# DJjjjhao/FIRA-ICSE

Hardware: AMD Instinct MI355X
Metric: training commits/sec (FIRA default config) (higher is better)
Workload: dtype f32; 1 GPU; BASELINE configs[1]: FIRA training step (fwd+bwd+Adam, dropout 0.1/0.2), batch 32 commits/GPU, fp32, 650-node graphs (mean nnz 1066/graph), vocab 24650; global_batch=32, parallelism=dp1

## Files before the change

### fira_icse_amd/csrc/engine.h

```cpp
#pragma once
#include "common.h"
#include <string>
#include <vector>

namespace fira {

int gemm_f32(hipStream_t s, int tA, int tB, int M, int N, int K, const float* A, int lda, const float* B, int ldb,
             float* C, int ldc, const float* bias, int flags, int splitk);
int gemm_f32_ex(hipStream_t s, int tA, int tB, int M, int N, int K, const float* A, int lda, const float* B, int ldb,
                float* C, int ldc, const float* bias, int flags, int splitk, float* colsum,
                const int32_t* c_rows = nullptr, const float* relu_mask = nullptr);
int gemm_bf16_ex(hipStream_t s, int tA, int tB, int M, int N, int K, const float* A, int lda, const float* B, int ldb,
                 float* C, int ldc, const float* bias, int flags, int splitk, float* colsum,
                 const int32_t* c_rows = nullptr, const float* relu_mask = nullptr);
struct ShadowEntry { int64_t offset; int rows, cols, pitch_t; int64_t offset_t; };
constexpr int SHADOW_MAX = 64;
struct ShadowTable {
    int n = 0;
    int64_t wbt_elems = 0;
    int tile_start[SHADOW_MAX + 1] = {0};
    ShadowEntry e[SHADOW_MAX];
};
int weight_shadows(hipStream_t s, const ShadowTable& tab, const float* P, uint16_t* Wb, uint16_t* WbT);
int gemm_bf16_wb_ex(hipStream_t s, int M, int N, int K, const float* A, int lda, const uint16_t* Bb, int ldb, float* C,
                    int ldc, const float* bias, int flags, int splitk, const int32_t* c_rows = nullptr,
                    const float* relu_mask = nullptr);
int gemm_bf16_group_add_wgrad(hipStream_t s, int M, int N, int K, const float* A, int lda, const float* B, int ldb,
                              float* C, int ldc, float* colsum, int max_split = 0);
int gemm_bf16_group_flush(hipStream_t s);
bool gemm_bf16_takes(int M, int N, int K);
void gemm_bf16_group_reset();
bool gemm_bf16_group_full();
bool gemm_wgrad_panel_takes(int M, int N, int K, const float* A, int lda, const float* B, int ldb, int ldc);
void gemm_wgrad_panel_reset();
bool gemm_wgrad_panel_full();
int gemm_wgrad_panel_pending();
int gemm_wgrad_panel_add(int M, int N, int K, const float* A, int lda, const float* B, int ldb, float* C, int ldc, float* colsum);
int gemm_wgrad_panel_flush(hipStream_t s, int np);
void gemm_wgrad_panel_scratch(float* buf, size_t n_floats);
int gemm_wgrad_panel(hipStream_t s, int np, int M, int N, int K, const float* A, int lda, const float* B, int ldb, float* C,
                     int ldc, float* colsum);
int gemm_group_add_wgrad(hipStream_t s, int M, int N, int K, const float* A, int lda, const float* B, int ldb, float* C,
                         int ldc, float* colsum, int max_split = 0);
int gemm_group_flush(hipStream_t s);
void gemm_group_reset();
bool gemm_group_full();
void gemm_set_pad_stream(hipStream_t s);
struct EpiRes;
bool gemm_tile32_takes(int tB, int M, int N, int K, const float* A, int lda, const float* B, int ldb);
bool gemm_tile32_try(hipStream_t s, int tB, int M, int N, int K, const float* A, int lda, const float* B, int ldb,
                     float* C, int ldc, const float* bias, int flags, int* rc, const int32_t* c_rows,
                     const float* relu_mask, const int32_t* a_rows, const EpiRes* er);
bool gemm_tile32_ln_try(hipStream_t s, int M, int N, const float* S, int lds, const float* W, const float* bias, float* Y,
                        int ldy, int flags, const float* gamma, const float* beta, float* x_out, float* stats_out, int* rc);
int gemm_tile32_lnb_blocks(int M);
bool gemm_tile32_lnb_try(hipStream_t s, int M, int N, const float* dy, const float* W, int ldw, float* dX, int lddx,
                         const float* relu_mask, const float* sum, const float* stats, const float* gamma, float* ds,
                         float* dx_drop, float* part, float dropout, uint64_t seed, uint32_t site, int* rc,
                         uint32_t idx0 = 0);
bool gemm_small_try(hipStream_t s, int tA, int tB, int M, int N, int K, const float* A, int lda, const float* B, int ldb,
                    float* C, int ldc, const float* bias, int flags, int* rc, const int32_t* c_rows = nullptr,
                    const float* relu_mask = nullptr);
int csr_spmm(hipStream_t s, int n_rows, const int32_t* rowptr, const int32_t* col, const float* val, const float* X,
             int ldx, float* Y, int ldy, int graph_rows, int variant);
int csr_spmm_ex(hipStream_t s, int n_rows, const int32_t* rowptr, const int32_t* col, const float* val, const float* X,
                int ldx, float* Y, int ldy, int graph_rows, int variant, int accum, float* rowsum);
int gcn_fused_fwd(hipStream_t s, int n_rows, const int32_t* rowptr, const int32_t* col, const float* val, const float* X,
                  const float* Wk, const float* bias, const float* r1_col, const float* gamma, const float* beta, float* sum,
                  float* y, float* stats, float* rowsum_out, const int32_t* slot2, float* y2, float dropout, uint64_t seed,
                  uint32_t site, int bf16, const uint16_t* Wx = nullptr);
int gcn_fused_bwd(hipStream_t s, int n_rows, const int32_t* rowptr, const int32_t* col, const float* val, const float* dY,
                  const float* Wk, float* u_out, float* acc_out, int bf16, const uint16_t* Wx = nullptr);
int gcn_split_planes(hipStream_t s, int n, const float* const* src, uint16_t* const* dst);
size_t head_logits_x3_scratch_elems(int R);
int head_logits_x3(hipStream_t s, int R, int V, const float* x, int ldx, const float* W, const float* bias, float* out, int ldo,
                   uint16_t* xplanes);
int transpose256(hipStream_t s, int nl, const float* W, float* Wt);
int linear_x3(hipStream_t s, int M, const float* X, int ldx, const uint16_t* Wx, int nb, const float* bias, float* out, int ldo,
              bool one_plane);
int split_planes_t(hipStream_t s, const float* W, int V, uint16_t* planes, bool one_plane);
int dgrad_x3_splitk(hipStream_t s, int M, int K, const float* A, int lda, const uint16_t* Wx, float* out, int ldo, bool one_plane);
int linear_x3_kacc(hipStream_t s, int M, const float* A, int lda, const uint16_t* Wx, int nkb, float* out, int ldo, bool accum,
                   bool one_plane);
int comb_fused_fwd(hipStream_t s, int n_rows, const float* Xc, const float* WqT, const float* WkT, const float* WoT,
                   const float* bqk, const float* bo, const float* vtab, int ldv, const int32_t* mark, float* qk, float* c,
                   const float* gamma, const float* beta, float* sum, float* y, const int32_t* y_rows, float* stats,
                   float dropout, uint64_t seed, uint32_t site_gate, uint32_t site_out, int bf16, const uint16_t* Wx = nullptr);
int comb_fused_bwd_parts();
int comb_fused_bwd(hipStream_t s, int n_rows, float* dG, const int32_t* rows, const float* sum, const float* stats,
                   const float* gamma, const float* Wo, const float* Wqk, const float* qk, const float* vtab, int ldv,
                   const int32_t* mark, float* dYc, float* dqk, float* part_ln, float* part_v, float dropout, uint64_t seed,
                   uint32_t site_gate, uint32_t site_out, int bf16, const uint16_t* WTx = nullptr);
struct TransposeTable { int n = 0; const float* src[24]; float* dst[24]; };
int transpose256_table(hipStream_t s, const TransposeTable& tab);
int embed_gather_fwd(hipStream_t s, int B, int L, const int32_t* idx, const float* table, const float* pos, float* out,
                     int out_bstride, int out_off);
int embed_grouped_bwd(hipStream_t s, int n_items, const int32_t* item_tok, const int32_t* item_ptr, const int32_t* rows,
                      float* dtable, const float* dnode);
int embed_list_bwd_small(hipStream_t s, int n, const int32_t* rows, const int32_t* ids, float* dtable, const float* dnode,
                         int table_rows);
int embed_gather_bwd(hipStream_t s, int B, int L, const int32_t* idx, float* dtable, const float* dout,
                     int out_bstride, int out_off, int padding_idx);
int embed_gather_bwd_small(hipStream_t s, int B, int L, const int32_t* idx, float* dtable, const float* dout,
                           int out_bstride, int out_off, int padding_idx, int table_rows);
int combination_fwd(hipStream_t s, int M, const float* qk, const float* vtab, int ldv, const int32_t* mark, float* out,
                    float dropout, uint64_t seed, uint32_t site);
int combination_bwd(hipStream_t s, int M, const float* qk, const float* vtab, int ldv, const int32_t* mark,
                    const float* dout, float* dqk, float* dvtab, int lddv, float dropout, uint64_t seed, uint32_t site,
                    float* part = nullptr);
int combination_bwd_blocks(int M);
struct RedEntry { float* dst; const float* src; int width, n_part, stride; };
constexpr int RED_MAX = 96;
struct RedTable {
    int n = 0;
    int wg_start[RED_MAX + 1] = {0};
    RedEntry e[RED_MAX];
};
int deferred_reduce(hipStream_t s, RedTable& tab);
int add_layernorm_fwd(hipStream_t s, int M, float* x, const float* res, const float* gamma, const float* beta,
                      float* y, float* stats, float dropout, uint64_t seed, uint32_t site, const int32_t* y_rows, const float* r1_row = nullptr,
                      const float* r1_col = nullptr,
                      const int32_t* slot2 = nullptr, float* y2 = nullptr,
// ... 170 lines not shown
```

### fira_icse_amd/csrc/engine.hip

```cpp
#include "engine.h"
#include <hip/hip_ext.h>
#include "epilogue.h"
#include <stdlib.h>
#include <map>
#include <mutex>

namespace fira {

static int64_t shadow_wbt_elems(const Layout& L);

struct Arena {
    char* base;
    size_t used = 0;
    explicit Arena(void* b) : base((char*)b) {}
    template <typename T>
    T* get(size_t n) {
        size_t bytes = (n * sizeof(T) + 255) / 256 * 256;
        T* p = base ? (T*)(base + used) : nullptr;
        used += bytes;
        return p;
    }
    float* f(size_t n) { return get<float>(n); }
};

// ... 45 lines not shown
    float* red_buf = nullptr;
    size_t red_cap = 0;
    float* panel_scratch = nullptr;
    size_t panel_floats = 0;
    float *dmem_c, *dsrc, *dsrc_c, *dtgt, *dkv_all, *ddec, *ddec_c, *dT_a, *dT_c;

    size_t build(void* ws, const fira_dims& d, int B_, bool training) {
        Arena a(ws);
        B = B_; L = d.sou_len; S = d.sub_len; A = d.ast_len; T = d.tar_len; V = d.vocab; nl = d.n_layer; F = d.d_ff;
        N = L + S + A;
        NB = B * N; CB = B * L; MB = B * (L + S); TB = B * T;
        ldl = (V + 63) / 64 * 64;
        const size_t D = FIRA_D;
        pos_code = a.f((size_t)L * D);
        pos_tar = a.f((size_t)T * D);
        mem_valid = a.get<int32_t>((size_t)MB);
        tar_valid = a.get<int32_t>((size_t)TB);
        compact_row = a.get<int32_t>((size_t)TB);
        iota = a.get<int32_t>((size_t)TB);
        row_bt = a.get<int32_t>((size_t)TB);
        rows_c = a.get<int32_t>((size_t)TB);
        code_slot = a.get<int32_t>((size_t)NB);
        mem_slot = a.get<int32_t>((size_t)NB);
        mem_off = a.get<int32_t>((size_t)B + 1);
        mem_valid_c = a.get<int32_t>((size_t)MB);
        inv_ntok = a.f(64);
        {
            const Layout* lay = get_layout(&d);
            const size_t tot = lay ? (size_t)lay->total : 0;
            wb = a.get<uint16_t>(tot);
            wbt = a.get<uint16_t>((lay ? (size_t)shadow_wbt_elems(*lay) : 0) + 64);
            w21b = a.get<uint16_t>((size_t)nl * D * D);
            w21bt = a.get<uint16_t>((size_t)nl * D * D + 64);
        }
        X.resize(nl + 1);
        for (int l = 0; l <= nl; ++l) X[l] = a.f((size_t)NB * D);
        enc.resize(nl);
        for (int l = 0; l < nl; ++l) {
            EncSave& e = enc[l];
            e.Xc = a.f((size_t)CB * D); e.qk = a.f((size_t)CB * 2 * D); e.c = a.f((size_t)CB * D);
            e.s1 = a.f((size_t)CB * D); e.st1 = a.f((size_t)CB * 2);
            e.Z = a.f((size_t)NB * D); e.s2 = a.f((size_t)NB * D); e.st2 = a.f((size_t)NB * 2);
        }
        vtab_all = a.f((size_t)4 * nl * D);
        W21 = a.f((size_t)nl * D * D); c21 = a.f((size_t)nl * D); rsum = a.f((size_t)NB);
        W21t = a.f((size_t)nl * D * D);
        W21x = a.get<uint16_t>((size_t)nl * 3 * D * D);
        W21tx = a.get<uint16_t>((size_t)nl * 3 * D * D);
        WcX = a.get<uint16_t>((size_t)nl * 9 * D * D);
        WcTX = a.get<uint16_t>((size_t)nl * 9 * D * D);
        WkvX = a.get<uint16_t>((size_t)nl * 6 * D * D);
        WkvT = a.f((size_t)nl * 2 * D * D);
        WkvTX = a.get<uint16_t>((size_t)nl * 6 * D * D);
        WoutTX = a.get<uint16_t>((size_t)cdiv(V, D) * 3 * D * D);
        xh_planes = a.get<uint16_t>(head_logits_x3_scratch_elems(TB));
        WcT = a.f((size_t)nl * 3 * D * D);
        H = a.f((size_t)NB * D);
        mem = a.f((size_t)MB * D);
        mem_c = a.f((size_t)MB * D);
        src_c = a.f((size_t)MB * D);
        x0 = a.f((size_t)TB * D);
        kvp = nl * 2 * D + KV_ROW_PAD;
        kv_all = a.f((size_t)MB * kvp);
        dec.resize(nl);
        for (int l = 0; l < nl; ++l) {
            DecSave& e = dec[l];
            e.qkv = a.f((size_t)TB * 3 * D); e.ao = a.f((size_t)TB * D); e.s_a = a.f((size_t)TB * D);
            e.st_a = a.f((size_t)TB * 2); e.x_a = a.f((size_t)TB * D); e.qc = a.f((size_t)TB * D);
            e.ao2 = a.f((size_t)TB * D); e.s_c = a.f((size_t)TB * D); e.st_c = a.f((size_t)TB * 2);
            e.x_c = a.f((size_t)TB * D); e.h = a.f((size_t)TB * F); e.s_f = a.f((size_t)TB * D);
            e.st_f = a.f((size_t)TB * 2); e.x_f = a.f((size_t)TB * D);
        }
        src = a.f((size_t)MB * D); tgt = a.f((size_t)TB * D);
        score = a.f((size_t)TB * (L + S)); gate = a.f((size_t)TB * 2);
        dec_c = a.f((size_t)TB * D); logits = a.f((size_t)TB * ldl);
        if (training) {
            dXa = a.f((size_t)NB * D); dXb = a.f((size_t)NB * D); dNB2 = a.f((size_t)NB * D);
            dCB_a = a.f((size_t)CB * D);
            red_cap = (size_t)nl * ((size_t)cdiv(NB, 16) * 4 * D + (size_t)cdiv(CB, 16) * 2 * D)
                    + (size_t)3 * nl * cdiv(TB, 16) * 2 * D
                    + (size_t)nl * std::max((size_t)cdiv(CB, 16) * 4 * D, (size_t)comb_fused_bwd_parts() * 6 * D + 64)
                    + (size_t)cdiv(L + S, 16) * B * COPY_PART_STRIDE + 4096;
            red_buf = a.f(red_cap);
            panel_floats = (size_t)320 * 256 * 256;
            panel_scratch = a.f(panel_floats);
            zero_beg = (float*)a.get<char>(0);
            dvtab_all = a.f((size_t)4 * nl * D);
            dW21 = a.f((size_t)nl * D * D + (size_t)nl * D); dc21 = dW21 + (size_t)nl * D * D;
            dtgt = a.f((size_t)TB * D);
            ddec_c = a.f((size_t)TB * D);
            zero_end = (float*)a.get<char>(0);
            dmem_c = a.f((size_t)MB * D); dsrc = a.f((size_t)MB * D); dsrc_c = a.f((size_t)MB * D);
            dkv_all = a.f((size_t)MB * kvp);
            ddec = a.f((size_t)TB * D);
            dT_a = a.f((size_t)TB * D); dT_c = a.f((size_t)TB * D);
            encg.resize(nl);
            decg.resize(nl);
            for (int l = 0; l < nl; ++l) {
                EncGrad& g = encg[l];
                g.dY2 = a.f((size_t)NB * D); g.dYc = a.f((size_t)CB * D);
                g.dqk = a.f((size_t)CB * 2 * D);
                DecGrad& h = decg[l];
                h.dYf = a.f((size_t)TB * D); h.dh = a.f((size_t)TB * F); h.dYc = a.f((size_t)TB * D);
                h.dq = a.f((size_t)TB * D); h.dYs = a.f((size_t)TB * D); h.dqkv = a.f((size_t)TB * 3 * D);
            }
        }
        return a.used;
    }
};

#define TRY(x)                 \
    do {                       \
        if (int e__ = (x)) return e__; \
    } while (0)

static int zero(hipStream_t s, void* p, size_t bytes) {
    hipError_t e = hipMemsetAsync(p, 0, bytes, s);
    if (e != hipSuccess) return set_err("hipMemsetAsync: %s", hipGetErrorString(e));
    return 0;
}

static thread_local int g_dtype = 0;
static thread_local int g_lanes = 1;
struct DtypeScope {
    int prev;
    explicit DtypeScope(int d) : prev(g_dtype) { g_dtype = d; }
    ~DtypeScope() { g_dtype = prev; }
};
static thread_local const float* g_P = nullptr;
static thread_local int64_t g_total = 0;
static thread_local const uint16_t* g_Wb = nullptr;
static thread_local const uint16_t* g_WbT = nullptr;
static thread_local const ShadowTable* g_tab = nullptr;
static thread_local const float* g_W21 = nullptr;
static thread_local int64_t g_W21n = 0;
static thread_local const uint16_t* g_W21b = nullptr;
static thread_local const uint16_t* g_W21bT = nullptr;

static const ShadowTable* shadow_table(const Layout& L) {
    static std::mutex mu;
    static std::map<const Layout*, ShadowTable*> cache;
    std::lock_guard<std::mutex> g(mu);
    auto it = cache.find(&L);
    if (it != cache.end()) return it->second;
    ShadowTable* t = new ShadowTable();
    const int D = FIRA_D;
    auto add = [&](int64_t off, int rows, int cols) {
        if (t->n == SHADOW_MAX) return;
        const int pitch = (rows + 7) / 8 * 8;
        t->e[t->n] = ShadowEntry{off, rows, cols, pitch, t->wbt_elems};
        t->wbt_elems += ((int64_t)cols * pitch + 63) / 64 * 64;
        t->tile_start[t->n + 1] = t->tile_start[t->n] + cdiv(rows, 64) * cdiv(cols, 64);
        ++t->n;
    };
    for (int l = 0; l < L.d.n_layer; ++l) {
        add(L.enc[l].wqk, 2 * D, D);
        add(L.enc[l].wo, D, D);
        add(L.dec[l].wqkv, 3 * D, D);
        add(L.dec[l].wo_s, D, D);
        add(L.dec[l].wq_c, D, D);
        add(L.dec[l].wo_c, D, D);
        add(L.dec[l].w1, L.d.d_ff, D);
        add(L.dec[l].w2, D, L.d.d_ff);
    }
    add(L.wkv_all, L.d.n_layer * 2 * D, D);
    add(L.wout, L.d.vocab, D);
    add(L.ws, D, D);
    add(L.wt, D, D);
// ... 1776 lines not shown
```

### fira_icse_amd/csrc/gemm_wgrad_panel.hip

```cpp
#include "engine.h"
#include "epilogue.h"
#include <algorithm>
#include <stdlib.h>

namespace fira {

typedef __bf16 pbf16x8 __attribute__((ext_vector_type(8)));
typedef __bf16 pbf16x2 __attribute__((ext_vector_type(2)));
typedef float pf32x2 __attribute__((ext_vector_type(2)));
typedef float pf32x16 __attribute__((ext_vector_type(16)));

constexpr int PN_T = 256;
constexpr int PN_KB = 16;
constexpr int PN_PART = PN_T * 32;
constexpr int PANEL_MAX = 48;

struct PanelProblem {
    const float *A, *B;
    float *C, *colsum;
    float* part;
    int M, N, K, lda, ldb, ldc;
    int tiles_m, tiles_n, slabs, k_slab;
};
struct PanelTable {
    int n;
    int wg_start[PANEL_MAX + 1];
    PanelProblem p[PANEL_MAX];
};

__device__ __forceinline__ int pn_unit(int row, int kh) { return kh * PN_T + row; }

__device__ __forceinline__ uint32_t pn_pack(float a, float b) {
    pf32x2 v = {a, b};
    return __builtin_bit_cast(uint32_t, __builtin_convertvector(v, pbf16x2));
}
__device__ __forceinline__ void pn_rest(float& a, float& b, uint32_t pk) {
    a -= __builtin_bit_cast(float, pk << 16);
    b -= __builtin_bit_cast(float, pk & 0xffff0000u);
}

__device__ __forceinline__ void pn_barrier() { asm volatile("s_waitcnt lgkmcnt(0)\n\ts_barrier" ::: "memory"); }

template <int NP>
__global__ __launch_bounds__(512) void wgrad_panel_kernel(const PanelTable tab) {
    extern __shared__ __attribute__((aligned(16))) char pn_lds[];
    __shared__ float pn_cs[PN_T];
    const int t = threadIdx.x, lane = t & 63, wave = __builtin_amdgcn_readfirstlane(t >> 6);
    int pi = 0;
    while (pi + 1 < tab.n && (int)blockIdx.x >= tab.wg_start[pi + 1]) ++pi;
    const PanelProblem& q = tab.p[pi];
    int w = blockIdx.x - tab.wg_start[pi];
    const int z = w % q.slabs;
    w /= q.slabs;
    const int tn = w % q.tiles_n, tm = w / q.tiles_n;
    const int m0 = tm * PN_T, n0 = tn * PN_T;
    const int k_beg = z * q.k_slab, k_end = min(q.K, k_beg + q.k_slab);
    const int nstep = (k_end - k_beg + PN_KB - 1) / PN_KB;
    const int opnd = t >> 8, idx = t & 255, kb = idx >> 7, cb = idx & 127;
    const float* src = opnd ? q.B : q.A;
    const int ld = opnd ? q.ldb : q.lda;
    const int c0 = (opnd ? n0 : m0) + 2 * cb;
    const int c_lim = opnd ? q.N : q.M;
    (void)c_lim;
    const rsrc_t rs = buf_rsrc(src, (unsigned)min((long)k_end * ld * 4, 0x7fffffffL));
    pf32x2 v0[8], v1[8];
    auto fetch = [&](int step, pf32x2 (&v)[8]) __attribute__((always_inline)) {
        const unsigned off0 = ((unsigned)(k_beg + step * PN_KB + kb * 8) * (unsigned)ld + (unsigned)c0) * 4u;
#pragma unroll
        for (int j = 0; j < 8; ++j) {
            const uint64_t raw = __builtin_bit_cast(uint64_t, __builtin_amdgcn_raw_buffer_load_b64(rs, off0 + (unsigned)j * (unsigned)ld * 4u, 0, 0));
            v[j] = __builtin_bit_cast(pf32x2, raw);
        }
    };
    float cs0 = 0.f, cs1 = 0.f;
    const bool do_cs = q.colsum != nullptr && tn == 0 && opnd == 0;
    char* const my_lds = pn_lds + opnd * (NP * PN_PART);
    const bool odd_first = (cb >> 2) & 1;
    const int u_first = pn_unit(2 * cb + (odd_first ? 1 : 0), kb) << 4, u_second = pn_unit(2 * cb + (odd_first ? 0 : 1), kb) << 4;
    auto put = [&](int buf, const pf32x2 (&v)[8]) __attribute__((always_inline)) {
        char* base = my_lds + buf * (2 * NP * PN_PART);
        float a[8], b[8];
#pragma unroll
        for (int j = 0; j < 8; ++j) { a[j] = v[j].x; b[j] = v[j].y; }
        if (do_cs) {
#pragma unroll
            for (int j = 0; j < 8; ++j) { cs0 += a[j]; cs1 += b[j]; }
        }
#pragma unroll
        for (int part = 0; part < NP; ++part) {
            uint4 wa, wb;
            wa.x = pn_pack(a[0], a[1]); wa.y = pn_pack(a[2], a[3]); wa.z = pn_pack(a[4], a[5]); wa.w = pn_pack(a[6], a[7]);
            wb.x = pn_pack(b[0], b[1]); wb.y = pn_pack(b[2], b[3]); wb.z = pn_pack(b[4], b[5]); wb.w = pn_pack(b[6], b[7]);
            const uint4 w_first = odd_first ? wb : wa, w_second = odd_first ? wa : wb;
            *reinterpret_cast<uint4*>(base + part * PN_PART + u_first) = w_first;
            *reinterpret_cast<uint4*>(base + part * PN_PART + u_second) = w_second;
            if (part + 1 < NP) {
                pn_rest(a[0], a[1], wa.x); pn_rest(a[2], a[3], wa.y); pn_rest(a[4], a[5], wa.z); pn_rest(a[6], a[7], wa.w);
                pn_rest(b[0], b[1], wb.x); pn_rest(b[2], b[3], wb.y); pn_rest(b[4], b[5], wb.z); pn_rest(b[6], b[7], wb.w);
            }
        }
    };
    const int wm = wave >> 2, wn = wave & 3;
    const int l31 = lane & 31, kh = lane >> 5;
    int offA[4], offB[2];
#pragma unroll
    for (int i = 0; i < 4; ++i) offA[i] = pn_unit(wm * 128 + i * 32 + l31, kh) << 4;
#pragma unroll
    for (int j = 0; j < 2; ++j) offB[j] = NP * PN_PART + (pn_unit(wn * 64 + j * 32 + l31, kh) << 4);
    pf32x16 acc[4][2];
#pragma unroll
    for (int i = 0; i < 4; ++i)
#pragma unroll
        for (int j = 0; j < 2; ++j)
#pragma unroll
            for (int r = 0; r < 16; ++r) acc[i][j][r] = 0.f;
    pbf16x8 a[NP][4], b[NP][2];
    auto frags = [&](int buf) __attribute__((always_inline)) {
        const char* base = pn_lds + buf * (2 * NP * PN_PART);
#pragma unroll
        for (int part = 0; part < NP; ++part) {
#pragma unroll
            for (int i = 0; i < 4; ++i) a[part][i] = *reinterpret_cast<const pbf16x8*>(base + part * PN_PART + offA[i]);
#pragma unroll
            for (int j = 0; j < 2; ++j) b[part][j] = *reinterpret_cast<const pbf16x8*>(base + part * PN_PART + offB[j]);
        }
    };
    auto compute = [&]() __attribute__((always_inline)) {
#pragma unroll
        for (int pr = (NP == 3 ? 0 : 5); pr < 6; ++pr) {
            const int pa = NP == 3 ? ((0x201100 >> (4 * (5 - pr))) & 3) : 0;
            const int pb = NP == 3 ? ((0x021010 >> (4 * (5 - pr))) & 3) : 0;
#pragma unroll
            for (int i = 0; i < 4; ++i)
#pragma unroll
                for (int j = 0; j < 2; ++j)
                    acc[i][j] = __builtin_amdgcn_mfma_f32_32x32x16_bf16(a[pa][i], b[pb][j], acc[i][j], 0, 0, 0);
        }
    };
    if (nstep > 0) {
        fetch(0, v0);
        fetch(1, v1);
        put(0, v0);
        fetch(2, v0);
        pn_barrier();
        for (int s = 0; s < nstep; s += 2) {
            put(1, v1);
            fetch(s + 2 + 1, v1);
            frags(0);
            compute();
            pn_barrier();
            put(0, v0);
            fetch(s + 2 + 2, v0);
            if (s + 1 < nstep) { frags(1); compute(); }
            pn_barrier();
        }
    }
    if (q.colsum != nullptr && tn == 0) {
        for (int i = t; i < PN_T; i += 512) pn_cs[i] = 0.f;
        __syncthreads();
        if (opnd == 0) { atomicAdd(&pn_cs[2 * cb], cs0); atomicAdd(&pn_cs[2 * cb + 1], cs1); }
        __syncthreads();
        for (int i = t; i < PN_T; i += 512)
            if (m0 + i < q.M) unsafeAtomicAdd(&q.colsum[m0 + i], pn_cs[i]);
    }
    if (q.slabs > 1) {
        float* pt = q.part + ((size_t)(tm * q.tiles_n + tn) * q.slabs + z) * (PN_T * PN_T);
#pragma unroll
        for (int j = 0; j < 2; ++j)
#pragma unroll
            for (int i = 0; i < 4; ++i)
#pragma unroll
                for (int r = 0; r < 16; ++r)
                    pt[(wm * 128 + i * 32 + (r & 3) + 8 * (r >> 2) + 4 * kh) * PN_T + wn * 64 + j * 32 + l31] = acc[i][j][r];
        return;
    }
    const rsrc_t rC = buf_rsrc(q.C, 0x7fffffffu);
#pragma unroll
    for (int j = 0; j < 2; ++j) {
        const int col = n0 + wn * 64 + j * 32 + l31;
#pragma unroll
        for (int i = 0; i < 4; ++i) {
            unsigned off[16];
            float old[16];
#pragma unroll
            for (int r = 0; r < 16; ++r) {
                const int row = m0 + wm * 128 + i * 32 + (r & 3) + 8 * (r >> 2) + 4 * kh;
                off[r] = (row < q.M && col < q.N) ? ((unsigned)row * (unsigned)q.ldc + (unsigned)col) * 4u : FIRA_OOB;
                old[r] = buf_load_f32(rC, off[r]);
            }
#pragma unroll
            for (int r = 0; r < 16; ++r)
                __builtin_amdgcn_raw_buffer_store_b32(__builtin_bit_cast(unsigned, old[r] + acc[i][j][r]), rC, off[r], 0, 0);
        }
    }
}

__global__ __launch_bounds__(256) void wgrad_panel_reduce_kernel(const PanelTable tab) {
    int b = blockIdx.x, pi = 0;
    for (pi = 0; pi < tab.n; ++pi) {
        const PanelProblem& q = tab.p[pi];
        if (q.slabs <= 1) continue;
        const int nb = q.tiles_m * q.tiles_n * 64;
        if (b < nb) break;
        b -= nb;
    }
    if (pi >= tab.n) return;
    const PanelProblem& q = tab.p[pi];
    const int tile = b >> 6, idx = (b & 63) * 256 + threadIdx.x;
    const int tm = tile / q.tiles_n, tn = tile % q.tiles_n;
    const int row = tm * PN_T + (idx >> 6), col = tn * PN_T + (idx & 63) * 4;
    const float4* pt = reinterpret_cast<const float4*>(q.part + (size_t)tile * q.slabs * (PN_T * PN_T)) + idx;
    float4 a = make_float4(0.f, 0.f, 0.f, 0.f);
    int z = 0;
    for (; z + 4 <= q.slabs; z += 4) {
        const float4 x0 = pt[(size_t)z * (PN_T * PN_T / 4)], x1 = pt[(size_t)(z + 1) * (PN_T * PN_T / 4)];
        const float4 x2 = pt[(size_t)(z + 2) * (PN_T * PN_T / 4)], x3 = pt[(size_t)(z + 3) * (PN_T * PN_T / 4)];
        a.x += (x0.x + x1.x) + (x2.x + x3.x); a.y += (x0.y + x1.y) + (x2.y + x3.y);
        a.z += (x0.z + x1.z) + (x2.z + x3.z); a.w += (x0.w + x1.w) + (x2.w + x3.w);
    }
    for (; z < q.slabs; ++z) {
        const float4 x = pt[(size_t)z * (PN_T * PN_T / 4)];
        a.x += x.x; a.y += x.y; a.z += x.z; a.w += x.w;
    }
    if (row >= q.M || col >= q.N) return;
    float4* c = reinterpret_cast<float4*>(q.C + (size_t)row * q.ldc + col);
    if ((((uintptr_t)c) & 15) == 0) {
        float4 o = *c;
        o.x += a.x; o.y += a.y; o.z += a.z; o.w += a.w;
        *c = o;
    } else {
        float* cf = reinterpret_cast<float*>(c);
        cf[0] += a.x; cf[1] += a.y; cf[2] += a.z; cf[3] += a.w;
    }
}

struct PanelBuilder {
    PanelTable t;
    PanelBuilder() { t.n = 0; t.wg_start[0] = 0; }
};
static PanelBuilder& panel() { static thread_local PanelBuilder b; return b; }

bool gemm_wgrad_panel_takes(int M, int N, int K, const float* A, int lda, const float* B, int ldb, int ldc) {
    return M >= 32 && N >= PN_T && N % PN_T == 0 && K >= 1 && lda % 2 == 0 && ldb % 2 == 0 &&
           ((uintptr_t)A % 8) == 0 && ((uintptr_t)B % 8) == 0 && (long)K * lda * 4 < 0x7fffffffL && (long)K * ldb * 4 < 0x7fffffffL &&
           epilogue_fits(M, ldc);
}
void gemm_wgrad_panel_reset() { panel().t.n = 0; }
bool gemm_wgrad_panel_full() { return panel().t.n == PANEL_MAX; }
int gemm_wgrad_panel_pending() { return panel().t.n; }

int gemm_wgrad_panel_add(int M, int N, int K, const float* A, int lda, const float* B, int ldb, float* C, int ldc, float* colsum) {
    PanelTable& t = panel().t;
    FIRA_REQUIRE(t.n < PANEL_MAX, "gemm_wgrad_panel_add: queue full (flush first)");
    PanelProblem& q = t.p[t.n++];
    q.A = A; q.B = B; q.C = C; q.colsum = colsum;
    q.M = M; q.N = N; q.K = K; q.lda = lda; q.ldb = ldb; q.ldc = ldc;
    q.tiles_m = cdiv(M, PN_T); q.tiles_n = N / PN_T;
    q.slabs = 1; q.k_slab = K; q.part = nullptr;
    return 0;
}
static thread_local float* g_panel_scratch = nullptr;
static thread_local size_t g_panel_scratch_floats = 0;
void gemm_wgrad_panel_scratch(float* buf, size_t n_floats) { g_panel_scratch = buf; g_panel_scratch_floats = n_floats; }
int gemm_wgrad_panel_flush(hipStream_t s, int np) {
    PanelTable& t = panel().t;
    if (t.n == 0) return 0;
    constexpr int target_wgs = 256;
    double work = 0, flop = 0, bytes = 0;
    for (int i = 0; i < t.n; ++i) {
        const PanelProblem& q = t.p[i];
        work += (double)q.tiles_m * q.tiles_n * q.K;
        flop += 2.0 * q.M * q.N * (double)q.K;
        bytes += 4.0 * ((double)q.M * q.K + (double)q.N * q.K + (double)q.M * q.N);
    }
    int tiles_total = 0;
    for (int i = 0; i < t.n; ++i) tiles_total += t.p[i].tiles_m * t.p[i].tiles_n;
    int per = std::max(256, (int)((work / target_wgs + PN_KB - 1) / PN_KB) * PN_KB);
    if (3 * tiles_total >= target_wgs) per = 1 << 30;
    size_t need = 0;
    for (int pass = 0; pass < 8; ++pass) {
        need = 0;
        for (int i = 0; i < t.n; ++i) {
            PanelProblem& q = t.p[i];
            q.slabs = g_panel_scratch ? std::max(1, cdiv(q.K, per)) : 1;
            q.k_slab = cdiv(cdiv(q.K, q.slabs), PN_KB) * PN_KB;
            q.slabs = cdiv(q.K, q.k_slab);
            if (q.slabs > 1) need += (size_t)q.tiles_m * q.tiles_n * q.slabs * (PN_T * PN_T);
        }
        if (need <= g_panel_scratch_floats) break;
        per *= 2;
    }
    if (need > g_panel_scratch_floats) {
        for (int i = 0; i < t.n; ++i) { t.p[i].slabs = 1; t.p[i].k_slab = cdiv(t.p[i].K, PN_KB) * PN_KB; }
        need = 0;
    }
    size_t off = 0;
    int bands = 0;
    for (int i = 0; i < t.n; ++i) {
        PanelProblem& q = t.p[i];
        q.part = nullptr;
        if (q.slabs > 1) {
            q.part = g_panel_scratch + off;
            off += (size_t)q.tiles_m * q.tiles_n * q.slabs * (PN_T * PN_T);
            bands += q.tiles_m * q.tiles_n * 64;
        }
        t.wg_start[i + 1] = t.wg_start[i] + q.tiles_m * q.tiles_n * q.slabs;
    }
    ProfScope prof(s, PROF_GEMM, flop, bytes);
    const size_t lds = (size_t)2 * 2 * np * PN_PART;
    static bool attr_set[2] = {false, false};
    if (np == 3) {
        if (!attr_set[1]) { (void)hipFuncSetAttribute((const void*)wgrad_panel_kernel<3>, hipFuncAttributeMaxDynamicSharedMemorySize, (int)lds); attr_set[1] = true; }
        hipLaunchKernelGGL(wgrad_panel_kernel<3>, dim3(t.wg_start[t.n]), dim3(512), lds, s, t);
    } else {
        if (!attr_set[0]) { (void)hipFuncSetAttribute((const void*)wgrad_panel_kernel<1>, hipFuncAttributeMaxDynamicSharedMemorySize, (int)lds); attr_set[0] = true; }
        hipLaunchKernelGGL(wgrad_panel_kernel<1>, dim3(t.wg_start[t.n]), dim3(512), lds, s, t);
    }
    if (bands > 0) hipLaunchKernelGGL(wgrad_panel_reduce_kernel, dim3(bands), dim3(256), 0, s, t);
    t.n = 0;
    FIRA_CHECK_LAUNCH("wgrad_panel");
    return 0;
}
int gemm_wgrad_panel(hipStream_t s, int np, int M, int N, int K, const float* A, int lda, const float* B, int ldb, float* C,
                     int ldc, float* colsum) {
    FIRA_REQUIRE(panel().t.n == 0, "gemm_wgrad_panel: problems are queued (flush first)");
    if (int rc = gemm_wgrad_panel_add(M, N, K, A, lda, B, ldb, C, ldc, colsum)) return rc;
    return gemm_wgrad_panel_flush(s, np);
}

}

extern "C" int fira_gemm_wgrad_panel(void* stream, int dtype, int M, int N, int K, const float* A, int lda, const float* B, int ldb,
                                     float* C, int ldc, float* colsum, float* scratch, size_t scratch_floats) {
    FIRA_REQUIRE(A && B && C && (dtype == 0 || dtype == 1), "fira_gemm_wgrad_panel: bad argument");
    FIRA_REQUIRE(fira::gemm_wgrad_panel_takes(M, N, K, A, lda, B, ldb, ldc),
                 "fira_gemm_wgrad_panel: shape %d x %d x %d / alignment not taken (M >= 32, N %% 256 == 0, even pitches)", M, N, K);
    fira::gemm_wgrad_panel_scratch(scratch, scratch ? scratch_floats : 0);
    const int rc = fira::gemm_wgrad_panel((hipStream_t)stream, dtype == 1 ? 1 : 3, M, N, K, A, lda, B, ldb, C, ldc, colsum);
    fira::gemm_wgrad_panel_scratch(nullptr, 0);
    return rc;
}
```

Measured before the change: 13410 commits/s.

## Add 128-wide tile variant to wgrad panel GEMM and re-plan split-K

Templates the grouped weight-gradient panel kernel on tile size, adding a 128x128 tile variant with 256 threads alongside the 256x256 one. A new planner picks 128 tiles when there are too few 256 tiles to fill the CUs, and uses split-K with 256 tiles only when the grid is under-filled or K is large. Problems are launched as two sub-tables, one per tile size. The split-K scratch buffer is now sized from a host-side plan of the expected problem sets instead of a fixed constant. This aims to raise occupancy for small wgrad batches, at the cost of an extra launch and lower per-tile reuse with 128 tiles.

```diff
diff --git a/fira_icse_amd/csrc/engine.h b/fira_icse_amd/csrc/engine.h
--- a/fira_icse_amd/csrc/engine.h
+++ b/fira_icse_amd/csrc/engine.h
@@ -38,6 +38,7 @@
 int gemm_wgrad_panel_add(int M, int N, int K, const float* A, int lda, const float* B, int ldb, float* C, int ldc, float* colsum);
 int gemm_wgrad_panel_flush(hipStream_t s, int np);
 void gemm_wgrad_panel_scratch(float* buf, size_t n_floats);
+size_t gemm_wgrad_panel_plan_floats(int n, const int (*mnk)[3]);
 int gemm_wgrad_panel(hipStream_t s, int np, int M, int N, int K, const float* A, int lda, const float* B, int ldb, float* C,
                      int ldc, float* colsum);
 int gemm_group_add_wgrad(hipStream_t s, int M, int N, int K, const float* A, int lda, const float* B, int ldb, float* C,
diff --git a/fira_icse_amd/csrc/engine.hip b/fira_icse_amd/csrc/engine.hip
--- a/fira_icse_amd/csrc/engine.hip
+++ b/fira_icse_amd/csrc/engine.hip
@@ -151,8 +151,28 @@
                     + (size_t)nl * std::max((size_t)cdiv(CB, 16) * 4 * D, (size_t)comb_fused_bwd_parts() * 6 * D + 64)
                     + (size_t)cdiv(L + S, 16) * B * COPY_PART_STRIDE + 4096;
             red_buf = a.f(red_cap);
-            panel_floats = (size_t)320 * 256 * 256;
-            panel_scratch = a.f(panel_floats);
+            {
+                std::vector<int> q;
+                auto add = [&](int M, int N, int K) { q.push_back(M); q.push_back(N); q.push_back(K); };
+                auto ask = [&]() {
+                    const int n = std::min((int)q.size() / 3, 48);
+                    panel_floats = std::max(panel_floats, gemm_wgrad_panel_plan_floats(n, (const int (*)[3])q.data()));
+                    q.clear();
+                };
+                panel_floats = 0;
+                for (int g : {1, nl}) {
+                    for (int l = 0; l < g; ++l) { add(D, D, NB); add(D, D, CB); add(2 * D, D, CB); }
+                    ask();
+                }
+                for (int g : {std::min(3, nl), nl}) {
+                    for (int l = 0; l < g; ++l) { add(D, F, TB); add(F, D, TB); add(D, D, TB); add(D, D, TB); add(D, D, TB); add(3 * D, D, TB); }
+                    add(D, D, TB); add(D, D, MB);
+                    ask();
+                    add(g * 2 * D, D, MB);
+                    ask();
+                }
+            }
+            panel_scratch = a.f(std::max(panel_floats, (size_t)1));
             zero_beg = (float*)a.get<char>(0);
             dvtab_all = a.f((size_t)4 * nl * D);
             dW21 = a.f((size_t)nl * D * D + (size_t)nl * D); dc21 = dW21 + (size_t)nl * D * D;
diff --git a/fira_icse_amd/csrc/gemm_wgrad_panel.hip b/fira_icse_amd/csrc/gemm_wgrad_panel.hip
--- a/fira_icse_amd/csrc/gemm_wgrad_panel.hip
+++ b/fira_icse_amd/csrc/gemm_wgrad_panel.hip
@@ -10,9 +10,7 @@
 typedef float pf32x2 __attribute__((ext_vector_type(2)));
 typedef float pf32x16 __attribute__((ext_vector_type(16)));
 
-constexpr int PN_T = 256;
 constexpr int PN_KB = 16;
-constexpr int PN_PART = PN_T * 32;
 constexpr int PANEL_MAX = 48;
 
 struct PanelProblem {
@@ -20,6 +18,7 @@
     float *C, *colsum;
     float* part;
     int M, N, K, lda, ldb, ldc;
+    int ts;
     int tiles_m, tiles_n, slabs, k_slab;
 };
 struct PanelTable {
@@ -28,7 +27,8 @@
     PanelProblem p[PANEL_MAX];
 };
 
-__device__ __forceinline__ int pn_unit(int row, int kh) { return kh * PN_T + row; }
+template <int TS>
+__device__ __forceinline__ int pn_unit(int row, int kh) { return kh * TS + row; }
 
 __device__ __forceinline__ uint32_t pn_pack(float a, float b) {
     pf32x2 v = {a, b};
@@ -41,10 +41,14 @@
 
 __device__ __forceinline__ void pn_barrier() { asm volatile("s_waitcnt lgkmcnt(0)\n\ts_barrier" ::: "memory"); }
 
-template <int NP>
-__global__ __launch_bounds__(512) void wgrad_panel_kernel(const PanelTable tab) {
+template <int NP, int TS>
+__global__ __launch_bounds__(2 * TS) void wgrad_panel_kernel(const PanelTable tab) {
+    constexpr int NT = 2 * TS;
+    constexpr int PART = TS * 32;
+    constexpr int WN = TS / 64;
+    constexpr int AI = TS / 64;
     extern __shared__ __attribute__((aligned(16))) char pn_lds[];
-    __shared__ float pn_cs[PN_T];
+    __shared__ float pn_cs[TS];
     const int t = threadIdx.x, lane = t & 63, wave = __builtin_amdgcn_readfirstlane(t >> 6);
     int pi = 0;
     while (pi + 1 < tab.n && (int)blockIdx.x >= tab.wg_start[pi + 1]) ++pi;
@@ -53,15 +57,13 @@
     const int z = w % q.slabs;
     w /= q.slabs;
     const int tn = w % q.tiles_n, tm = w / q.tiles_n;
-    const int m0 = tm * PN_T, n0 = tn * PN_T;
+    const int m0 = tm * TS, n0 = tn * TS;
     const int k_beg = z * q.k_slab, k_end = min(q.K, k_beg + q.k_slab);
     const int nstep = (k_end - k_beg + PN_KB - 1) / PN_KB;
-    const int opnd = t >> 8, idx = t & 255, kb = idx >> 7, cb = idx & 127;
+    const int opnd = t / TS, idx = t & (TS - 1), kb = idx / (TS / 2), cb = idx & (TS / 2 - 1);
     const float* src = opnd ? q.B : q.A;
     const int ld = opnd ? q.ldb : q.lda;
     const int c0 = (opnd ? n0 : m0) + 2 * cb;
-    const int c_lim = opnd ? q.N : q.M;
-    (void)c_lim;
     const rsrc_t rs = buf_rsrc(src, (unsigned)min((long)k_end * ld * 4, 0x7fffffffL));
     pf32x2 v0[8], v1[8];
     auto fetch = [&](int step, pf32x2 (&v)[8]) __attribute__((always_inline)) {
@@ -74,11 +76,11 @@
     };
     float cs0 = 0.f, cs1 = 0.f;
     const bool do_cs = q.colsum != nullptr && tn == 0 && opnd == 0;
-    char* const my_lds = pn_lds + opnd * (NP * PN_PART);
+    char* const my_lds = pn_lds + opnd * (NP * PART);
     const bool odd_first = (cb >> 2) & 1;
-    const int u_first = pn_unit(2 * cb + (odd_first ? 1 : 0), kb) << 4, u_second = pn_unit(2 * cb + (odd_first ? 0 : 1), kb) << 4;
+    const int u_first = pn_unit<TS>(2 * cb + (odd_first ? 1 : 0), kb) << 4, u_second = pn_unit<TS>(2 * cb + (odd_first ? 0 : 1), kb) << 4;
     auto put = [&](int buf, const pf32x2 (&v)[8]) __attribute__((always_inline)) {
-        char* base = my_lds + buf * (2 * NP * PN_PART);
+        char* base = my_lds + buf * (2 * NP * PART);
         float a[8], b[8];
 #pragma unroll
         for (int j = 0; j < 8; ++j) { a[j] = v[j].x; b[j] = v[j].y; }
@@ -92,37 +94,37 @@
             wa.x = pn_pack(a[0], a[1]); wa.y = pn_pack(a[2], a[3]); wa.z = pn_pack(a[4], a[5]); wa.w = pn_pack(a[6], a[7]);
             wb.x = pn_pack(b[0], b[1]); wb.y = pn_pack(b[2], b[3]); wb.z = pn_pack(b[4], b[5]); wb.w = pn_pack(b[6], b[7]);
             const uint4 w_first = odd_first ? wb : wa, w_second = odd_first ? wa : wb;
-            *reinterpret_cast<uint4*>(base + part * PN_PART + u_first) = w_first;
-            *reinterpret_cast<uint4*>(base + part * PN_PART + u_second) = w_second;
+            *reinterpret_cast<uint4*>(base + part * PART + u_first) = w_first;
+            *reinterpret_cast<uint4*>(base + part * PART + u_second) = w_second;
             if (part + 1 < NP) {
                 pn_rest(a[0], a[1], wa.x); pn_rest(a[2], a[3], wa.y); pn_rest(a[4], a[5], wa.z); pn_rest(a[6], a[7], wa.w);
                 pn_rest(b[0], b[1], wb.x); pn_rest(b[2], b[3], wb.y); pn_rest(b[4], b[5], wb.z); pn_rest(b[6], b[7], wb.w);
             }
         }
     };
-    const int wm = wave >> 2, wn = wave & 3;
+    const int wm = wave / WN, wn = wave % WN;
     const int l31 = lane & 31, kh = lane >> 5;
-    int offA[4], offB[2];
-#pragma unroll
-    for (int i = 0; i < 4; ++i) offA[i] = pn_unit(wm * 128 + i * 32 + l31, kh) << 4;
-#pragma unroll
-    for (int j = 0; j < 2; ++j) offB[j] = NP * PN_PART + (pn_unit(wn * 64 + j * 32 + l31, kh) << 4);
-    pf32x16 acc[4][2];
-#pragma unroll
-    for (int i = 0; i < 4; ++i)
+    int offA[AI], offB[2];
+#pragma unroll
+    for (int i = 0; i < AI; ++i) offA[i] = pn_unit<TS>(wm * (TS / 2) + i * 32 + l31, kh) << 4;
+#pragma unroll
+    for (int j = 0; j < 2; ++j) offB[j] = NP * PART + (pn_unit<TS>(wn * 64 + j * 32 + l31, kh) << 4);
+    pf32x16 acc[AI][2];
+#pragma unroll
+    for (int i = 0; i < AI; ++i)
 #pragma unroll
         for (int j = 0; j < 2; ++j)
 #pragma unroll
             for (int r = 0; r < 16; ++r) acc[i][j][r] = 0.f;
-    pbf16x8 a[NP][4], b[NP][2];
+    pbf16x8 a[NP][AI], b[NP][2];
     auto frags = [&](int buf) __attribute__((always_inline)) {
-        const char* base = pn_lds + buf * (2 * NP * PN_PART);
+        const char* base = pn_lds + buf * (2 * NP * PART);
 #pragma unroll
         for (int part = 0; part < NP; ++part) {
 #pragma unroll
-            for (int i = 0; i < 4; ++i) a[part][i] = *reinterpret_cast<const pbf16x8*>(base + part * PN_PART + offA[i]);
-#pragma unroll
-            for (int j = 0; j < 2; ++j) b[part][j] = *reinterpret_cast<const pbf16x8*>(base + part * PN_PART + offB[j]);
+            for (int i = 0; i < AI; ++i) a[part][i] = *reinterpret_cast<const pbf16x8*>(base + part * PART + offA[i]);
+#pragma unroll
+            for (int j = 0; j < 2; ++j) b[part][j] = *reinterpret_cast<const pbf16x8*>(base + part * PART + offB[j]);
         }
     };
     auto compute = [&]() __attribute__((always_inline)) {
@@ -131,7 +133,7 @@
             const int pa = NP == 3 ? ((0x201100 >> (4 * (5 - pr))) & 3) : 0;
             const int pb = NP == 3 ? ((0x021010 >> (4 * (5 - pr))) & 3) : 0;
 #pragma unroll
-            for (int i = 0; i < 4; ++i)
+            for (int i = 0; i < AI; ++i)
 #pragma unroll
                 for (int j = 0; j < 2; ++j)
                     acc[i][j] = __builtin_amdgcn_mfma_f32_32x32x16_bf16(a[pa][i], b[pb][j], acc[i][j], 0, 0, 0);
@@ -156,22 +158,22 @@
         }
     }
     if (q.colsum != nullptr && tn == 0) {
-        for (int i = t; i < PN_T; i += 512) pn_cs[i] = 0.f;
+        for (int i = t; i < TS; i += NT) pn_cs[i] = 0.f;
         __syncthreads();
         if (opnd == 0) { atomicAdd(&pn_cs[2 * cb], cs0); atomicAdd(&pn_cs[2 * cb + 1], cs1); }
         __syncthreads();
-        for (int i = t; i < PN_T; i += 512)
+        for (int i = t; i < TS; i += NT)
             if (m0 + i < q.M) unsafeAtomicAdd(&q.colsum[m0 + i], pn_cs[i]);
     }
     if (q.slabs > 1) {
-        float* pt = q.part + ((size_t)(tm * q.tiles_n + tn) * q.slabs + z) * (PN_T * PN_T);
+        float* pt = q.part + ((size_t)(tm * q.tiles_n + tn) * q.slabs + z) * (TS * TS);
 #pragma unroll
         for (int j = 0; j < 2; ++j)
 #pragma unroll
-            for (int i = 0; i < 4; ++i)
+            for (int i = 0; i < AI; ++i)
 #pragma unroll
                 for (int r = 0; r < 16; ++r)
-                    pt[(wm * 128 + i * 32 + (r & 3) + 8 * (r >> 2) + 4 * kh) * PN_T + wn * 64 + j * 32 + l31] = acc[i][j][r];
+                    pt[(wm * (TS / 2) + i * 32 + (r & 3) + 8 * (r >> 2) + 4 * kh) * TS + wn * 64 + j * 32 + l31] = acc[i][j][r];
         return;
     }
     const rsrc_t rC = buf_rsrc(q.C, 0x7fffffffu);
@@ -179,12 +181,12 @@
     for (int j = 0; j < 2; ++j) {
         const int col = n0 + wn * 64 + j * 32 + l31;
 #pragma unroll
-        for (int i = 0; i < 4; ++i) {
+        for (int i = 0; i < AI; ++i) {
             unsigned off[16];
             float old[16];
 #pragma unroll
             for (int r = 0; r < 16; ++r) {
-                const int row = m0 + wm * 128 + i * 32 + (r & 3) + 8 * (r >> 2) + 4 * kh;
+                const int row = m0 + wm * (TS / 2) + i * 32 + (r & 3) + 8 * (r >> 2) + 4 * kh;
                 off[r] = (row < q.M && col < q.N) ? ((unsigned)row * (unsigned)q.ldc + (unsigned)col) * 4u : FIRA_OOB;
                 old[r] = buf_load_f32(rC, off[r]);
             }
@@ -200,26 +202,27 @@
     for (pi = 0; pi < tab.n; ++pi) {
         const PanelProblem& q = tab.p[pi];
         if (q.slabs <= 1) continue;
-        const int nb = q.tiles_m * q.tiles_n * 64;
+        const int nb = q.tiles_m * q.tiles_n * (q.ts * q.ts / 1024);
         if (b < nb) break;
         b -= nb;
     }
     if (pi >= tab.n) return;
     const PanelProblem& q = tab.p[pi];
-    const int tile = b >> 6, idx = (b & 63) * 256 + threadIdx.x;
+    const int ts = q.ts, per_tile = ts * ts / 1024, row_f4 = ts / 4, tile_f4 = ts * ts / 4;
+    const int tile = b / per_tile, idx = (b % per_tile) * 256 + threadIdx.x;
     const int tm = tile / q.tiles_n, tn = tile % q.tiles_n;
-    const int row = tm * PN_T + (idx >> 6), col = tn * PN_T + (idx & 63) * 4;
-    const float4* pt = reinterpret_cast<const float4*>(q.part + (size_t)tile * q.slabs * (PN_T * PN_T)) + idx;
+    const int row = tm * ts + idx / row_f4, col = tn * ts + (idx % row_f4) * 4;
+    const float4* pt = reinterpret_cast<const float4*>(q.part + (size_t)tile * q.slabs * (ts * ts)) + idx;
     float4 a = make_float4(0.f, 0.f, 0.f, 0.f);
     int z = 0;
     for (; z + 4 <= q.slabs; z += 4) {
-        const float4 x0 = pt[(size_t)z * (PN_T * PN_T / 4)], x1 = pt[(size_t)(z + 1) * (PN_T * PN_T / 4)];
-        const float4 x2 = pt[(size_t)(z + 2) * (PN_T * PN_T / 4)], x3 = pt[(size_t)(z + 3) * (PN_T * PN_T / 4)];
+        const float4 x0 = pt[(size_t)z * tile_f4], x1 = pt[(size_t)(z + 1) * tile_f4];
+        const float4 x2 = pt[(size_t)(z + 2) * tile_f4], x3 = pt[(size_t)(z + 3) * tile_f4];
         a.x += (x0.x + x1.x) + (x2.x + x3.x); a.y += (x0.y + x1.y) + (x2.y + x3.y);
         a.z += (x0.z + x1.z) + (x2.z + x3.z); a.w += (x0.w + x1.w) + (x2.w + x3.w);
     }
     for (; z < q.slabs; ++z) {
-        const float4 x = pt[(size_t)z * (PN_T * PN_T / 4)];
+        const float4 x = pt[(size_t)z * tile_f4];
         a.x += x.x; a.y += x.y; a.z += x.z; a.w += x.w;
     }
     if (row >= q.M || col >= q.N) return;
@@ -241,7 +244,7 @@
 static PanelBuilder& panel() { static thread_local PanelBuilder b; return b; }
 
 bool gemm_wgrad_panel_takes(int M, int N, int K, const float* A, int lda, const float* B, int ldb, int ldc) {
-    return M >= 32 && N >= PN_T && N % PN_T == 0 && K >= 1 && lda % 2 == 0 && ldb % 2 == 0 &&
+    return M >= 32 && N >= 256 && N % 256 == 0 && K >= 1 && lda % 2 == 0 && ldb % 2 == 0 &&
            ((uintptr_t)A % 8) == 0 && ((uintptr_t)B % 8) == 0 && (long)K * lda * 4 < 0x7fffffffL && (long)K * ldb * 4 < 0x7fffffffL &&
            epilogue_fits(M, ldc);
 }
@@ -255,68 +258,105 @@
     PanelProblem& q = t.p[t.n++];
     q.A = A; q.B = B; q.C = C; q.colsum = colsum;
     q.M = M; q.N = N; q.K = K; q.lda = lda; q.ldb = ldb; q.ldc = ldc;
-    q.tiles_m = cdiv(M, PN_T); q.tiles_n = N / PN_T;
+    q.ts = 128; q.tiles_m = cdiv(M, 128); q.tiles_n = N / 128;
     q.slabs = 1; q.k_slab = K; q.part = nullptr;
     return 0;
 }
+
+constexpr int PN_CUS = 256;
+constexpr int PN_MIN_SLAB = 256;
+constexpr int PN_SPLIT_TS = 256;
+static void pn_shape(PanelProblem& q, int ts) { q.ts = ts; q.tiles_m = cdiv(q.M, ts); q.tiles_n = q.N / ts; }
+static size_t panel_plan(PanelTable& t, bool may_split, size_t scratch_floats) {
+    double work = 0;
+    int tiles_big = 0, tiles_small = 0;
+    for (int i = 0; i < t.n; ++i) {
+        const PanelProblem& q = t.p[i];
+        work += (double)cdiv(q.M, 128) * (q.N / 128) * q.K;
+        tiles_small += cdiv(q.M, 128) * (q.N / 128);
+        tiles_big += cdiv(q.M, 256) * (q.N / 256);
+    }
+    const int ts_whole = tiles_big >= PN_CUS ? 256 : 128;
+    const bool under = tiles_small < PN_CUS;
+    int T = std::max(PN_KB, (int)((work / PN_CUS + PN_KB - 1) / PN_KB) * PN_KB);
+    size_t need = 0;
+    for (int pass = 0; pass < 8; ++pass) {
+        need = 0;
+        const int rows = std::max(PN_MIN_SLAB, cdiv(T / 4, PN_KB) * PN_KB);
+        for (int i = 0; i < t.n; ++i) {
+            PanelProblem& q = t.p[i];
+            constexpr int ts_split = PN_SPLIT_TS;
+            const bool split = may_split && q.K > rows && (under || q.K >= 2 * T);
+            pn_shape(q, split ? ts_split : ts_whole);
+            q.slabs = split ? cdiv(q.K, rows) : 1;
+            q.k_slab = cdiv(cdiv(q.K, q.slabs), PN_KB) * PN_KB;
+            q.slabs = cdiv(q.K, q.k_slab);
+            if (q.slabs > 1) need += (size_t)q.tiles_m * q.tiles_n * q.slabs * (q.ts * q.ts);
+        }
+        if (!may_split || need <= scratch_floats) break;
+        T *= 2;
+    }
+    if (need > scratch_floats) {
+        for (int i = 0; i < t.n; ++i) { PanelProblem& q = t.p[i]; pn_shape(q, ts_whole); q.slabs = 1; q.k_slab = cdiv(q.K, PN_KB) * PN_KB; }
+        need = 0;
+    }
+    return need;
+}
+size_t gemm_wgrad_panel_plan_floats(int n, const int (*mnk)[3]) {
+    PanelTable t;
+    t.n = std::min(n, PANEL_MAX);
+    for (int i = 0; i < t.n; ++i) { PanelProblem& q = t.p[i]; q.M = mnk[i][0]; q.N = mnk[i][1]; q.K = mnk[i][2]; }
+    return panel_plan(t, true, ~(size_t)0);
+}
+
 static thread_local float* g_panel_scratch = nullptr;
 static thread_local size_t g_panel_scratch_floats = 0;
 void gemm_wgrad_panel_scratch(float* buf, size_t n_floats) { g_panel_scratch = buf; g_panel_scratch_floats = n_floats; }
+
+template <int NP, int TS>
+static void panel_launch(hipStream_t s, const PanelTable& t) {
+    PanelTable sub;
+    sub.n = 0; sub.wg_start[0] = 0;
+    for (int i = 0; i < t.n; ++i) {
+        if (t.p[i].ts != TS) continue;
+        const PanelProblem& q = sub.p[sub.n] = t.p[i];
+        sub.wg_start[sub.n + 1] = sub.wg_start[sub.n] + q.tiles_m * q.tiles_n * q.slabs;
+        ++sub.n;
+    }
+    if (sub.n == 0) return;
+    constexpr size_t lds = (size_t)2 * 2 * NP * TS * 32;
+    static bool attr_set = false;
+    if (!attr_set) { (void)hipFuncSetAttribute((const void*)wgrad_panel_kernel<NP, TS>, hipFuncAttributeMaxDynamicSharedMemorySize, (int)lds); attr_set = true; }
+    hipLaunchKernelGGL((wgrad_panel_kernel<NP, TS>), dim3(sub.wg_start[sub.n]), dim3(2 * TS), lds, s, sub);
+}
 int gemm_wgrad_panel_flush(hipStream_t s, int np) {
     PanelTable& t = panel().t;
     if (t.n == 0) return 0;
-    constexpr int target_wgs = 256;
-    double work = 0, flop = 0, bytes = 0;
-    for (int i = 0; i < t.n; ++i) {
-        const PanelProblem& q = t.p[i];
-        work += (double)q.tiles_m * q.tiles_n * q.K;
-        flop += 2.0 * q.M * q.N * (double)q.K;
-        bytes += 4.0 * ((double)q.M * q.K + (double)q.N * q.K + (double)q.M * q.N);
-    }
-    int tiles_total = 0;
-    for (int i = 0; i < t.n; ++i) tiles_total += t.p[i].tiles_m * t.p[i].tiles_n;
-    int per = std::max(256, (int)((work / target_wgs + PN_KB - 1) / PN_KB) * PN_KB);
-    if (3 * tiles_total >= target_wgs) per = 1 << 30;
-    size_t need = 0;
-    for (int pass = 0; pass < 8; ++pass) {
-        need = 0;
-        for (int i = 0; i < t.n; ++i) {
-            PanelProblem& q = t.p[i];
-            q.slabs = g_panel_scratch ? std::max(1, cdiv(q.K, per)) : 1;
-            q.k_slab = cdiv(cdiv(q.K, q.slabs), PN_KB) * PN_KB;
-            q.slabs = cdiv(q.K, q.k_slab);
-            if (q.slabs > 1) need += (size_t)q.tiles_m * q.tiles_n * q.slabs * (PN_T * PN_T);
-        }
-        if (need <= g_panel_scratch_floats) break;
-        per *= 2;
-    }
-    if (need > g_panel_scratch_floats) {
-        for (int i = 0; i < t.n; ++i) { t.p[i].slabs = 1; t.p[i].k_slab = cdiv(t.p[i].K, PN_KB) * PN_KB; }
-        need = 0;
-    }
+    panel_plan(t, g_panel_scratch != nullptr, g_panel_scratch_floats);
+    double flop = 0, bytes = 0, part_bytes = 0;
     size_t off = 0;
     int bands = 0;
     for (int i = 0; i < t.n; ++i) {
         PanelProblem& q = t.p[i];
+        flop += 2.0 * q.M * q.N * (double)q.K;
+        bytes += 4.0 * ((double)q.M * q.K + (double)q.N * q.K + (double)q.M * q.N);
         q.part = nullptr;
         if (q.slabs > 1) {
             q.part = g_panel_scratch + off;
-            off += (size_t)q.tiles_m * q.tiles_n * q.slabs * (PN_T * PN_T);
-            bands += q.tiles_m * q.tiles_n * 64;
-        }
-        t.wg_start[i + 1] = t.wg_start[i] + q.tiles_m * q.tiles_n * q.slabs;
-    }
-    ProfScope prof(s, PROF_GEMM, flop, bytes);
-    const size_t lds = (size_t)2 * 2 * np * PN_PART;
-    static bool attr_set[2] = {false, false};
-    if (np == 3) {
-        if (!attr_set[1]) { (void)hipFuncSetAttribute((const void*)wgrad_panel_kernel<3>, hipFuncAttributeMaxDynamicSharedMemorySize, (int)lds); attr_set[1] = true; }
-        hipLaunchKernelGGL(wgrad_panel_kernel<3>, dim3(t.wg_start[t.n]), dim3(512), lds, s, t);
-    } else {
-        if (!attr_set[0]) { (void)hipFuncSetAttribute((const void*)wgrad_panel_kernel<1>, hipFuncAttributeMaxDynamicSharedMemorySize, (int)lds); attr_set[0] = true; }
-        hipLaunchKernelGGL(wgrad_panel_kernel<1>, dim3(t.wg_start[t.n]), dim3(512), lds, s, t);
-    }
-    if (bands > 0) hipLaunchKernelGGL(wgrad_panel_reduce_kernel, dim3(bands), dim3(256), 0, s, t);
+            off += (size_t)q.tiles_m * q.tiles_n * q.slabs * (q.ts * q.ts);
+            bands += q.tiles_m * q.tiles_n * (q.ts * q.ts / 1024);
+        }
+    }
+    part_bytes = 4.0 * (double)off;
+    {
+        ProfScope prof(s, PROF_GEMM, flop, bytes);
+        if (np == 3) { panel_launch<3, 128>(s, t); panel_launch<3, 256>(s, t); }
+        else { panel_launch<1, 128>(s, t); panel_launch<1, 256>(s, t); }
+    }
+    if (bands > 0) {
+        ProfScope prof(s, PROF_GEMM, 0.0, part_bytes);
+        hipLaunchKernelGGL(wgrad_panel_reduce_kernel, dim3(bands), dim3(256), 0, s, t);
+    }
     t.n = 0;
     FIRA_CHECK_LAUNCH("wgrad_panel");
     return 0;
```

After: 13410 commits/s, median of 3. Within noise of the previous version (+0.0%).
